# huangzh13/StyleGAN.pytorch

Measured on AMD Instinct MI355X. Metric: img/s full G+D train step, 1024x1024 depth-9 bf16, higher is better.
Workload: dtype bf16; 1 GPU; ffhq1024: StyleGAN 1024x1024, progressive depth index 8, logistic+R1, alpha 0.5, batch 4/GPU, global batch 4; global_batch=4, parallelism=dp1

## Files before the change

stylegan/pytorch_amd/csrc/conv.hip:

```cpp
#include "common.h"
#include <stdlib.h>

enum { G3X3 = 0, GDOWN = 1, GUP = 2, GUPA = 3 };

SGX_SWITCH(conv_percu_cap, "SGX_CONV_PERCU", 0)
SGX_SWITCH(conv_max_ct, "SGX_CONV_MAXCT", 4)
SGX_SWITCH(conv_max_bp, "SGX_CONV_MAXBP", 256)
SGX_SWITCH(conv_min_blocks_env, "SGX_CONV_MINBLOCKS", 0)
SGX_SWITCH(conv_deep_k_on, "SGX_CONV_DEEPK", 1)
SGX_SWITCH(conv_upa_on, "SGX_CONV_UPA", 1)
SGX_SWITCH(conv_splitk_env, "SGX_CONV_SPLITK", 1)
#ifdef SGX_PROBE_BUILD
SGX_SWITCH(conv_dbg, "SGX_CONV_DBG", 0)
#endif

template <typename T, int KC> struct Frag;
template <> struct Frag<float, 16> {
    static constexpr int NK = 4;
    static constexpr int rowb_w() { return 68; }
    static constexpr int rowb_in(int) { return 68; }
    static constexpr bool swz_w() { return false; }
    static constexpr bool swz_in(int) { return false; }
    typedef float frag_t;
    static constexpr int pad_pw(int pw, int) { return pw; }
// ... 574 lines not shown
    }
    SGX_REQUIRE(false, SGX_EINVAL, "conv: bad dtype %d", dtype);
}

__global__ __launch_bounds__(256) void conv_splitk_finish(const float* __restrict__ kws, int ksplit, size_t npix, int Cout, const float* __restrict__ bias,
                                                          int act, const bf16_t* __restrict__ mask, bf16_t* __restrict__ y) {
    const size_t nvec = npix * Cout / 8, stride = npix * Cout;
    const size_t i = (size_t)blockIdx.x * 256 + threadIdx.x;
    if (i >= nvec) return;
    const int c0 = (int)((i * 8) % Cout);
    float v[8];
#pragma unroll
    for (int j = 0; j < 8; ++j) v[j] = 0.f;
    for (int s = 0; s < ksplit; ++s) {
        const float4 a0 = *reinterpret_cast<const float4*>(kws + s * stride + i * 8), a1 = *reinterpret_cast<const float4*>(kws + s * stride + i * 8 + 4);
        v[0] += a0.x; v[1] += a0.y; v[2] += a0.z; v[3] += a0.w; v[4] += a1.x; v[5] += a1.y; v[6] += a1.z; v[7] += a1.w;
    }
    if (bias) {
#pragma unroll
        for (int j = 0; j < 8; ++j) v[j] += bias[c0 + j];
    }
    if (act == SGX_ACT_LRELU) {
#pragma unroll
        for (int j = 0; j < 8; ++j) v[j] = lrelu(v[j]);
    }
    uint4 o = make_uint4(pack_bf16x2(v[0], v[1]), pack_bf16x2(v[2], v[3]), pack_bf16x2(v[4], v[5]), pack_bf16x2(v[6], v[7]));
    if (mask) o = lrelu_mask_bf16x8(o, *reinterpret_cast<const uint4*>(mask + i * 8));
    *reinterpret_cast<uint4*>(y + i * 8) = o;
}
static int conv_splitk_plan(int geo, int B, int H, int W, int Cin, int Cout, int dtype) {
    const int on = conv_splitk_env() < 0 ? 1 : conv_splitk_env();
    if (!on || dtype != SGX_BF16 || geo < 0 || geo > 2 || Cin % 16 || Cout % 16) return 0;
    if (geo != GDOWN) return 0;
    if (sgx_conv2_takes(geo, B, H, W, Cin, Cout)) return 0;
    const int ohc = conv_tile_extent(geo, H), owc = conv_tile_extent(geo, W);
    const bool deep = geo != GDOWN && conv_deep_k(geo, B, ohc, owc, Cin, Cout);
    const ConvCfg c = pick_cfg((geo == GUP && !deep) ? GUPA : geo, B, ohc, owc, Cout);
    if (!c.bp || c.bp > 128 || c.ct > 2 || (deep && c.ct != 1)) return 0;
    const int kc = deep ? 128 : (Cin % 32 == 0 ? 32 : 16);
    const int nk = Cin / kc;
    const long blocks = (long)((B + c.ni - 1) / c.ni) * ((ohc + c.th - 1) / c.th) * ((owc + c.tw - 1) / c.tw) * (Cout / (16 * c.ct)) * ((geo == GUP && deep) ? 4 : 1);
    const int ncu = sgx_ncu();
    if (nk < 4 || blocks > ncu) return 0;
    int want = (int)((2L * ncu + blocks - 1) / blocks);
    const int cap = on > 1 ? on : 8;
    if (want > cap) want = cap;
    if (want > nk / 2) want = nk / 2;
    return want >= 2 ? want : 0;
}
extern "C" size_t sgx_conv_splitk_ws_bytes(int geo, int B, int H, int W, int Cin, int Cout, int dtype) {
    const int ks = conv_splitk_plan(geo, B, H, W, Cin, Cout, dtype);
    if (!ks) return 0;
    const size_t opix = (size_t)B * sgx_conv_out(geo, H) * sgx_conv_out(geo, W);
    return (size_t)ks * opix * Cout * sizeof(float);
}
extern "C" int sgx_conv_splitk(int geo, const void* x, const void* w, const float* bias, void* y, const void* mask, int B, int H, int W, int Cin, int Cout,
                               int act, int dtype, void* ws, size_t ws_bytes, void* stream) {
    const int ks = conv_splitk_plan(geo, B, H, W, Cin, Cout, dtype);
    SGX_REQUIRE(ks > 1, SGX_EUNSUPPORTED, "conv_splitk: this shape does not split (geo %d B%d %dx%d %d->%d)", geo, B, H, W, Cin, Cout);
    SGX_REQUIRE(x && w && y && ws && ws_bytes >= sgx_conv_splitk_ws_bytes(geo, B, H, W, Cin, Cout, dtype), SGX_EWORKSPACE, "conv_splitk: workspace");
    SGX_REQUIRE(geo == G3X3 || !mask, SGX_EINVAL, "conv_splitk: the output mask belongs to the 3x3 geometry");
    SGX_REQUIRE(geo != GDOWN || (H % 2 == 0 && W % 2 == 0), SGX_EINVAL, "conv_splitk: odd input size");
    hipStream_t st = (hipStream_t)stream;
    ConvArgs a = conv_args(geo, x, w, nullptr, y, B, H, W, Cin, Cout, SGX_ACT_NONE);
    a.ksplit = ks; a.kws = static_cast<float*>(ws);
    const int OH = a.OH, OW = a.OW;
    const double taps = geo == G3X3 ? 9.0 : 16.0, opix = (double)B * OH * OW, macs = geo == GUP ? taps / 4.0 : taps;
    SGX_NOTE(2.0 * macs * Cin * Cout * opix, 2.0 * ((double)B * H * W * Cin + opix * Cout + taps * Cin * Cout) + 4.0 * ks * opix * Cout, "conv%c/k%d B%d %dx%d %d->%d",
             geo == G3X3 ? 'S' : (geo == GDOWN ? 'D' : 'U'), ks, B, H, W, Cin, Cout);
    int rc;
    SGX_REQUIRE(geo == GDOWN, SGX_EUNSUPPORTED, "conv_splitk: only the stride-2 geometry has split-K kernels");
    rc = dispatch_conv<GDOWN, true>(a, dtype, st);
    if (rc) return rc;
    const size_t npix = (size_t)B * OH * OW, nvec = npix * Cout / 8;
    SGX_NOTE(0.0, 4.0 * ks * npix * Cout + 2.0 * npix * Cout, "conv_splitk_finish %zux%d", npix, Cout);
    hipLaunchKernelGGL(conv_splitk_finish, dim3((unsigned)((nvec + 255) / 256)), dim3(256), 0, st, (const float*)ws, ks, npix, Cout, bias, act,
                       static_cast<const bf16_t*>(mask), static_cast<bf16_t*>(y));
    SGX_LAUNCH_CHECK("conv_splitk_finish");
    return 0;
}

extern "C" int sgx_conv_config(int geo, int B, int H, int W, int Cin, int Cout, int dtype, int* cfg5) {
    SGX_REQUIRE(geo >= 0 && geo <= 2 && cfg5, SGX_EINVAL, "conv_config: bad args");
    const int ohc = conv_tile_extent(geo, H), owc = conv_tile_extent(geo, W);
    const ConvCfg c = pick_cfg(geo, B, ohc, owc, Cout);
    cfg5[0] = dtype == SGX_F32 ? 16 : (conv_deep_k(geo, B, ohc, owc, Cin, Cout) ? 128 : (Cin % 32 == 0 ? 32 : 16));
    cfg5[1] = c.th; cfg5[2] = c.tw; cfg5[3] = c.bp; cfg5[4] = c.ct;
    return 0;
}

template <int GEO>
static int conv_forward(ConvArgs& a, int dtype, hipStream_t st) {
    if (dtype == SGX_BF16) {
        int launched = 0;
        const int rc = sgx_conv2_try(GEO, a.x, a.w, a.bias, a.y, a.B, a.H, a.W, a.Cin, a.Cout, a.act, a.mask, -1, st, &launched);
        if (rc || launched) return rc;
    }
    return dispatch_conv<GEO>(a, dtype, st);
}

extern "C" int sgx_conv3x3(const void* x, const void* w, const float* bias, void* y, int B, int H, int W, int Cin,
                           int Cout, int act, const void* mask, int dtype, void* stream) {
    ConvArgs a = conv_args(G3X3, x, w, bias, y, B, H, W, Cin, Cout, act);
    a.mask = mask;
    const double es = dtype == SGX_F32 ? 4 : 2;
    SGX_NOTE(2.0 * 9 * Cin * Cout * B * H * W, es * ((double)B * H * W * (Cin + Cout) + 9.0 * Cin * Cout), "convS B%d %dx%d %d->%d", B, H, W, Cin, Cout);
    return conv_forward<G3X3>(a, dtype, (hipStream_t)stream);
}

extern "C" int sgx_conv4x4s2_down(const void* x, const void* w, const float* bias, void* y, int B, int H, int W,
                                  int Cin, int Cout, int act, int dtype, void* stream) {
    SGX_REQUIRE(H % 2 == 0 && W % 2 == 0, SGX_EINVAL, "conv4x4s2_down: odd input size");
    ConvArgs a = conv_args(GDOWN, x, w, bias, y, B, H, W, Cin, Cout, act);
    const double es = dtype == SGX_F32 ? 4 : 2;
    SGX_NOTE(2.0 * 16 * Cin * Cout * B * (H / 2) * (W / 2), es * ((double)B * H * W * (Cin + Cout / 4.0) + 16.0 * Cin * Cout), "convD B%d %dx%d %d->%d", B, H, W, Cin, Cout);
    return conv_forward<GDOWN>(a, dtype, (hipStream_t)stream);
}

extern "C" int sgx_conv4x4s2_up(const void* x, const void* w, void* y, int B, int H, int W, int Cin, int Cout,
                                int dtype, void* stream) {
    ConvArgs a = conv_args(GUP, x, w, nullptr, y, B, H, W, Cin, Cout, SGX_ACT_NONE);
    const double es = dtype == SGX_F32 ? 4 : 2;
    SGX_NOTE(2.0 * 16 * Cin * Cout * B * H * W, es * ((double)B * H * W * (Cin + 4.0 * Cout) + 16.0 * Cin * Cout), "convU B%d %dx%d %d->%d", B, H, W, Cin, Cout);
    return conv_forward<GUP>(a, dtype, (hipStream_t)stream);
}

extern "C" int sgx_conv_variant(int geo, const void* x, const void* w, const float* bias, void* y, int B, int H, int W, int Cin,
                                int Cout, int act, int dtype, int variant, void* stream) {
    SGX_REQUIRE(geo >= 0 && geo <= 2, SGX_EINVAL, "conv_variant: bad geometry %d", geo);
    SGX_REQUIRE(geo != GDOWN || (H % 2 == 0 && W % 2 == 0), SGX_EINVAL, "conv_variant: odd input size");
    SGX_REQUIRE(geo != GUP || (!bias && act == SGX_ACT_NONE), SGX_EINVAL, "conv_variant: the transposed convolution has no fused bias / activation");
    ConvArgs a = conv_args(geo, x, w, bias, y, B, H, W, Cin, Cout, act);
    const int OH = a.OH, OW = a.OW;
    const double es = dtype == SGX_F32 ? 4 : 2, taps = geo == G3X3 ? 9 : 16, npix = (double)B * (geo == GDOWN ? OH * OW : H * W);
    SGX_NOTE(2.0 * taps * Cin * Cout * npix, es * ((double)B * (H * W * Cin + OH * OW * Cout) + taps * Cin * Cout), "conv%c/v%d B%d %dx%d %d->%d", "SDU"[geo], variant, B, H, W, Cin, Cout);
    if (variant == 0) {
        if (geo == G3X3) return dispatch_conv<G3X3>(a, dtype, (hipStream_t)stream);
        if (geo == GDOWN) return dispatch_conv<GDOWN>(a, dtype, (hipStream_t)stream);
        return dispatch_conv<GUP>(a, dtype, (hipStream_t)stream);
    }
    SGX_REQUIRE(dtype == SGX_BF16 && (variant == 4 || variant == 8 || (variant >= 20 && variant <= 29) || (variant >= 30 && variant <= 36)), SGX_EINVAL,
                "conv_variant: variant %d needs bf16 and 4 or 8 waves (or 20..29: a wide-block configuration, 30..36: a conv3_kernel configuration)", variant);
    int launched = 0;
    const int rc = sgx_conv2_try(geo, x, w, bias, y, B, H, W, Cin, Cout, act, nullptr, variant, (hipStream_t)stream, &launched);
    SGX_REQUIRE(rc || launched, SGX_EUNSUPPORTED, "conv_variant: shape not covered by the second-generation kernel");
    return rc;
}

struct WgradArgs {
    const void* kside; const void* nside; float* out;
    int B, Hk, Wk, Hn, Wn, Ck, Cn, tiles_x, tiles_y, ntiles;
    int want_bias;
    int direct; float* dw; float* db; int O, I, mode, transposed, flip_t, accumulate; float scale;
};

template <typename T> struct WFrag;
template <> struct WFrag<float> {
    static constexpr int KPS = 4;
    static constexpr int row_bytes(int ch) { return (ch == 16 ? 16 : ch + 16) * 4; }
    typedef float frag_t;
    __device__ static __forceinline__ frag_t load(const char* base, const int (&poff)[4], int q, int choff) {
        return *reinterpret_cast<const float*>(base + poff[0] + choff * 4);
    }
    __device__ static __forceinline__ f32x4 mma(frag_t a, frag_t b, f32x4 c) {
        return __builtin_amdgcn_mfma_f32_16x16x4f32(a, b, c, 0, 0, 0);
    }
    __device__ static __forceinline__ frag_t ones() { return 1.f; }
};
template <> struct WFrag<bf16_t> {
    static constexpr int KPS = 16;
    static constexpr int row_bytes(int ch) { return ch * 2 + 16; }
    typedef s16x4 frag_t;
    __device__ static __forceinline__ frag_t load(const char* base, const int (&poff)[4], int q, int choff) {
        s16x4 r;
#pragma unroll
        for (int j = 0; j < 4; ++j) r[j] = *reinterpret_cast<const short*>(base + poff[j] + choff * 2);
        return r;
    }
    __device__ static __forceinline__ f32x4 mma(frag_t a, frag_t b, f32x4 c) {
        return __builtin_amdgcn_mfma_f32_16x16x16bf16_1k(a, b, c, 0, 0, 0);
    }
    __device__ static __forceinline__ frag_t ones() { return (s16x4){0x3f80, 0x3f80, 0x3f80, 0x3f80}; }
};

__device__ __forceinline__ s16x4 lds_tr16(const char* p) {
    return __builtin_amdgcn_ds_read_tr16_b64_v4i16((s16x4 __attribute__((address_space(3)))*)(p));
}
__device__ __forceinline__ bf16x8 cat8(s16x4 lo, s16x4 hi) {
    typedef __attribute__((ext_vector_type(8))) short s16x8;
    s16x8 v = __builtin_shufflevector(lo, hi, 0, 1, 2, 3, 4, 5, 6, 7);
    return __builtin_bit_cast(bf16x8, v);
}

template <typename T>
constexpr int wgrad_pitch(int ch, bool tr, int is) {
    return (tr && is == 1) ? (ch == 16 ? 32 : ch * 2 + 32) : WFrag<T>::row_bytes(ch);
}

template <typename T, int GEO, int TH, int TW, int BP, int NSUB, int KSUB, bool TR>
__global__ __launch_bounds__(256) void wgrad_kernel(WgradArgs a) {
    using F = WFrag<T>;
    constexpr int IS = Geo<GEO>::IS, TK = Geo<GEO>::TK, NT = TK * TK;
    constexpr int PH = (TH - 1) * IS + TK, PW = (TW - 1) * IS + TK;
    constexpr int NI = BP / (TH * TW);
    constexpr int NCH = NSUB * 16, KCH = KSUB * 16;
    constexpr int NROW = wgrad_pitch<T>(NCH, TR, 1), KROW = wgrad_pitch<T>(KCH, TR, IS);
    constexpr int VE = 16 / (int)sizeof(T);
    constexpr int TPW = (NT + 3) / 4;
    constexpr int PPL = F::KPS / 4;
    extern __shared__ __attribute__((aligned(16))) char smem[];
    char* n_lds = smem;
    char* k_lds = smem + BP * NROW;

    const int tid = threadIdx.x, lane = tid & 63, wave = tid >> 6, q = lane >> 4, l15 = lane & 15;
    const int kblocks = a.Ck / KCH;
    const int n0 = (blockIdx.x / kblocks) * NCH, kc0 = (blockIdx.x % kblocks) * KCH;
    const T* __restrict__ kg = static_cast<const T*>(a.kside);
    const T* __restrict__ ng = static_cast<const T*>(a.nside);

    f32x4 acc[TPW][NSUB][KSUB];
#pragma unroll
    for (int i = 0; i < TPW; ++i)
#pragma unroll
        for (int j = 0; j < NSUB; ++j)
#pragma unroll
            for (int k = 0; k < KSUB; ++k) acc[i][j][k] = (f32x4){0.f, 0.f, 0.f, 0.f};

    const bool do_bias = a.want_bias && (blockIdx.x % kblocks) == 0 && wave == 3;
    f32x4 bacc[NSUB];
#pragma unroll
    for (int j = 0; j < NSUB; ++j) bacc[j] = (f32x4){0.f, 0.f, 0.f, 0.f};

    constexpr int NNV = (BP * (NCH / VE) + 255) / 256, NKV = (NI * PH * PW * (KCH / VE) + 255) / 256;
    uint4 rn[NNV], rk[NKV];
    auto gload = [&](int tile) {
        int bx = tile;
        const int tx_i = bx % a.tiles_x; bx /= a.tiles_x;
        const int ty_i = bx % a.tiles_y;
        const int img0 = (bx / a.tiles_y) * NI;
        const int ty0 = ty_i * TH, tx0 = tx_i * TW;
        const int iy0 = ty0 * IS - 1, ix0 = tx0 * IS - 1;
#pragma unroll
        for (int j = 0; j < NNV; ++j) {
            const int idx = tid + j * 256;
            const int v = idx % (NCH / VE), m = idx / (NCH / VE);
            const int il = m / (TH * TW), r = (m / TW) % TH, c = m % TW;
            const int b = img0 + il, gy = ty0 + r, gx = tx0 + c;
            const bool ok = (idx < BP * (NCH / VE)) && (b < a.B) && (gy < a.Hn) && (gx < a.Wn);
            const T* src = ng + (((size_t)b * a.Hn + gy) * a.Wn + gx) * a.Cn + n0 + v * VE;
            rn[j] = ok ? *reinterpret_cast<const uint4*>(src) : make_uint4(0, 0, 0, 0);
        }
#pragma unroll
        for (int j = 0; j < NKV; ++j) {
            const int idx = tid + j * 256;
            const int v = idx % (KCH / VE), pixel = idx / (KCH / VE);
            const int il = pixel / (PH * PW), rem = pixel % (PH * PW);
            const int gy = iy0 + rem / PW, gx = ix0 + rem % PW, b = img0 + il;
            const bool ok = (idx < NI * PH * PW * (KCH / VE)) && (b < a.B) && ((unsigned)gy < (unsigned)a.Hk) && ((unsigned)gx < (unsigned)a.Wk);
            const T* src = kg + (((size_t)b * a.Hk + gy) * a.Wk + gx) * a.Ck + kc0 + v * VE;
            rk[j] = ok ? *reinterpret_cast<const uint4*>(src) : make_uint4(0, 0, 0, 0);
        }
    };
    auto lstore = [&]() {
#pragma unroll
        for (int j = 0; j < NNV; ++j) {
            const int idx = tid + j * 256;
            if (idx < BP * (NCH / VE)) *reinterpret_cast<uint4*>(n_lds + (idx / (NCH / VE)) * NROW + (idx % (NCH / VE)) * 16) = rn[j];
        }
#pragma unroll
        for (int j = 0; j < NKV; ++j) {
            const int idx = tid + j * 256;
            if (idx < NI * PH * PW * (KCH / VE)) *reinterpret_cast<uint4*>(k_lds + (idx / (KCH / VE)) * KROW + (idx % (KCH / VE)) * 16) = rk[j];
        }
    };
    if ((int)blockIdx.y < a.ntiles) gload(blockIdx.y);
    for (int tile = blockIdx.y; tile < a.ntiles; tile += gridDim.y) {
        __syncthreads();
        lstore();
        __syncthreads();
        if (tile + (int)gridDim.y < a.ntiles) gload(tile + gridDim.y);
        if constexpr (TR) {
            for (int ks = 0; ks < BP / 32; ++ks) {
                int noff2[2], koff2[2];
#pragma unroll
                for (int h = 0; h < 2; ++h) {
                    const int m = ks * 32 + h * 16 + q * 4 + (l15 >> 2);
                    const int il = m / (TH * TW), r = (m / TW) % TH, c = m % TW;
                    noff2[h] = m * NROW + (l15 & 3) * 8;
                    koff2[h] = ((il * PH + r * IS) * PW + c * IS) * KROW + (l15 & 3) * 8;
                }
                bf16x8 fa8[NSUB];
#pragma unroll
                for (int ns = 0; ns < NSUB; ++ns)
                    fa8[ns] = cat8(lds_tr16(n_lds + noff2[0] + ns * 32), lds_tr16(n_lds + noff2[1] + ns * 32));
                if (do_bias) {
                    const bf16x8 one8 = cat8(WFrag<bf16_t>::ones(), WFrag<bf16_t>::ones());
#pragma unroll
                    for (int ns = 0; ns < NSUB; ++ns) bacc[ns] = __builtin_amdgcn_mfma_f32_16x16x32_bf16(fa8[ns], one8, bacc[ns], 0, 0, 0);
                }
#pragma unroll
                for (int i = 0; i < TPW; ++i) {
                    const int t = wave + 4 * i;
                    if (t < NT) {
                        const int toff = ((t / TK) * PW + (t % TK)) * KROW;
#pragma unroll
                        for (int kk = 0; kk < KSUB; ++kk) {
                            const bf16x8 fb8 = cat8(lds_tr16(k_lds + toff + koff2[0] + kk * 32), lds_tr16(k_lds + toff + koff2[1] + kk * 32));
#pragma unroll
                            for (int ns = 0; ns < NSUB; ++ns)
                                acc[i][ns][kk] = __builtin_amdgcn_mfma_f32_16x16x32_bf16(fa8[ns], fb8, acc[i][ns][kk], 0, 0, 0);
                        }
                    }
                }
            }
        } else
        for (int ks = 0; ks < BP / F::KPS; ++ks) {
            int noff[4], koff[4];
#pragma unroll
            for (int j = 0; j < PPL; ++j) {
                const int m = ks * F::KPS + q * PPL + j;
                const int il = m / (TH * TW), r = (m / TW) % TH, c = m % TW;
                noff[j] = m * NROW;
                koff[j] = ((il * PH + r * IS) * PW + c * IS) * KROW;
            }
            typename F::frag_t fa[NSUB];
#pragma unroll
            for (int ns = 0; ns < NSUB; ++ns) fa[ns] = F::load(n_lds, noff, q, ns * 16 + l15);
            if (do_bias) {
#pragma unroll
                for (int ns = 0; ns < NSUB; ++ns) bacc[ns] = F::mma(fa[ns], F::ones(), bacc[ns]);
            }
#pragma unroll
            for (int i = 0; i < TPW; ++i) {
                const int t = wave + 4 * i;
                if (t < NT) {
                    const int toff = ((t / TK) * PW + (t % TK)) * KROW;
#pragma unroll
                    for (int kk = 0; kk < KSUB; ++kk) {
                        typename F::frag_t fb = F::load(k_lds + toff, koff, q, kk * 16 + l15);
#pragma unroll
                        for (int ns = 0; ns < NSUB; ++ns) acc[i][ns][kk] = F::mma(fa[ns], fb, acc[i][ns][kk]);
                    }
                }
            }
        }
    }
    if (a.direct) {
        constexpr int KP = KCH + 1;
        float* accl = reinterpret_cast<float*>(smem);
        __syncthreads();
#pragma unroll
        for (int i = 0; i < TPW; ++i) {
            const int t = wave + 4 * i;
            if (t < NT) {
#pragma unroll
                for (int ns = 0; ns < NSUB; ++ns)
#pragma unroll
                    for (int kk = 0; kk < KSUB; ++kk)
#pragma unroll
                        for (int r = 0; r < 4; ++r) accl[(t * NCH + ns * 16 + q * 4 + r) * KP + kk * 16 + l15] = acc[i][ns][kk][r];
            }
        }
        __syncthreads();
        const float c = a.scale * (a.mode == SGX_PACK_D ? 0.25f : 1.f);
        for (int idx = tid; idx < NCH * KCH * 9; idx += 256) {
            const int tap = idx % 9, kl = (idx / 9) % KCH, nl = idx / (9 * KCH);
            const int n = n0 + nl, k = kc0 + kl;
            const int o = a.transposed ? k : n, i = a.transposed ? n : k;
            if (i >= a.I || o >= a.O) continue;
            float v;
            if (NT == 9) {
                v = accl[((a.flip_t ? 8 - tap : tap) * NCH + nl) * KP + kl];
            } else {
                const int y = tap / 3, x = tap % 3;
                const float* pp = accl + nl * KP + kl;
                v = (pp[(y * 4 + x) * NCH * KP] + pp[(y * 4 + x + 1) * NCH * KP]) +
                    (pp[((y + 1) * 4 + x) * NCH * KP] + pp[((y + 1) * 4 + x + 1) * NCH * KP]);
            }
            float* d = a.dw + ((size_t)o * a.I + i) * 9 + (a.mode == SGX_PACK_UF ? 8 - tap : tap);
            *d = (a.accumulate & 1) ? *d + c * v : c * v;
        }
        if (do_bias && l15 == 0) {
#pragma unroll
            for (int ns = 0; ns < NSUB; ++ns)
#pragma unroll
                for (int r = 0; r < 4; ++r) {
                    float* d = a.db + n0 + ns * 16 + q * 4 + r;
                    *d = (a.accumulate & 2) ? *d + bacc[ns][r] : bacc[ns][r];
                }
        }
        return;
    }
    float* out = a.out + (size_t)blockIdx.y * ((size_t)NT * a.Cn * a.Ck + a.Cn);
    if (do_bias && l15 == 0) {
#pragma unroll
        for (int ns = 0; ns < NSUB; ++ns)
#pragma unroll
            for (int r = 0; r < 4; ++r) out[(size_t)NT * a.Cn * a.Ck + n0 + ns * 16 + q * 4 + r] = bacc[ns][r];
    }
#pragma unroll
    for (int i = 0; i < TPW; ++i) {
        const int t = wave + 4 * i;
        if (t < NT) {
#pragma unroll
            for (int ns = 0; ns < NSUB; ++ns)
#pragma unroll
                for (int kk = 0; kk < KSUB; ++kk)
#pragma unroll
                    for (int r = 0; r < 4; ++r)
                        out[((size_t)t * a.Cn + n0 + ns * 16 + q * 4 + r) * a.Ck + kc0 + kk * 16 + l15] = acc[i][ns][kk][r];
        }
    }
}

struct FinishArgs { const float* ws; float* dw; float* db; int nsplit, O, I, Ip, mode, transposed, flip_t; float scale; int accumulate; };

template <int EPB>
__global__ __launch_bounds__(256) void wgrad_finish_kernel(FinishArgs f) {
    constexpr int NSL = 256 / EPB;
    __shared__ float red[NSL][EPB][9];
    const int pl = threadIdx.x % EPB, sl = threadIdx.x / EPB;
    const int A = f.transposed ? f.Ip : f.O, Bd = f.transposed ? f.O : f.Ip;
    const int e = blockIdx.x * EPB + pl;
    const int taps = f.mode == SGX_PACK_S ? 9 : 16;
    const size_t tstride = (size_t)f.O * f.Ip, total = (size_t)taps * tstride + A;
    if ((int)blockIdx.x >= (A * Bd + EPB - 1) / EPB) {
        const int o = ((int)blockIdx.x - (A * Bd + EPB - 1) / EPB) * EPB + pl;
        float b = 0.f;
        if (o < f.O)
            for (int s = sl; s < f.nsplit; s += NSL) b += f.ws[(size_t)s * total + (size_t)taps * tstride + o];
        red[sl][pl][0] = b;
        __syncthreads();
        if (sl == 0 && o < f.O) {
            float sum = 0.f;
            for (int l = 0; l < NSL; ++l) sum += red[l][pl][0];
            f.db[o] = (f.accumulate & 2) ? f.db[o] + sum : sum;
        }
        return;
    }
    float acc[9];
#pragma unroll
    for (int k = 0; k < 9; ++k) acc[k] = 0.f;
    if (e < A * Bd) {
#pragma unroll 4
        for (int s = sl; s < f.nsplit; s += NSL) {
            const float* p = f.ws + (size_t)s * total + e;
            if (f.mode == SGX_PACK_S) {
#pragma unroll
                for (int t = 0; t < 9; ++t) acc[t] += p[(size_t)(f.flip_t ? 8 - t : t) * tstride];
            } else {
                float v[16];
#pragma unroll
                for (int t = 0; t < 16; ++t) v[t] = p[(size_t)t * tstride];
#pragma unroll
                for (int y = 0; y < 3; ++y)
#pragma unroll
                    for (int x = 0; x < 3; ++x)
                        acc[y * 3 + x] += (v[y * 4 + x] + v[y * 4 + x + 1]) + (v[(y + 1) * 4 + x] + v[(y + 1) * 4 + x + 1]);
            }
        }
    }
#pragma unroll
    for (int k = 0; k < 9; ++k) red[sl][pl][k] = acc[k];
    __syncthreads();
    for (int t = threadIdx.x; t < EPB * 9; t += 256) {
        const int el = t / 9, k = t % 9;
        const int ee = blockIdx.x * EPB + el;
        if (ee >= A * Bd) continue;
        const int a = ee / Bd, bb = ee % Bd;
        const int o = f.transposed ? bb : a, i = f.transposed ? a : bb;
        if (i >= f.I) continue;
        float sum = 0.f;
#pragma unroll 8
        for (int l = 0; l < NSL; ++l) sum += red[l][el][k];
        const float c = f.scale * (f.mode == SGX_PACK_D ? 0.25f : 1.f);
        float* d = f.dw + ((size_t)o * f.I + i) * 9 + (f.mode == SGX_PACK_UF ? 8 - k : k);
        *d = (f.accumulate & 1) ? *d + c * sum : c * sum;
    }
}

static int wgrad_nsplit(int pairs, int ntiles, size_t elems_per_split) {
    static const int env_target = [] { const char* e = getenv("SGX_WGRAD_BLOCKS"); return e && atoi(e) > 0 ? atoi(e) : 0; }();
    static const int env_cap = [] { const char* e = getenv("SGX_WGRAD_MAXSPLIT"); return e && atoi(e) > 0 ? atoi(e) : 0; }();
    const bool tiny = elems_per_split <= (size_t)16 * 32 * 32;
    static const int env_mid = [] { const char* e = getenv("SGX_WGRAD_BLOCKS_MID"); return e && atoi(e) > 0 ? atoi(e) : 0; }();
    const int target = env_target ? env_target : (tiny ? 2048 : (env_mid ? env_mid : 512)), cap = env_cap ? env_cap : (tiny ? 1024 : 512);
    int want = (target + pairs - 1) / pairs;
    if (!env_target && pairs >= 512 && ntiles <= 64) want = 1;
    if (want > cap) want = cap;
    if (want > ntiles) want = ntiles;
    if (want < 1) want = 1;
    return want;
}

template <typename T, int GEO, int TH, int TW, int BP, int NSUB, int KSUB, bool TR>
static int launch_wgrad(WgradArgs& a, void* ws, size_t ws_bytes, int* nsplit_out, hipStream_t st) {
    using F = WFrag<T>;
    constexpr int IS = Geo<GEO>::IS, TK = Geo<GEO>::TK, NT = TK * TK;
    constexpr int PH = (TH - 1) * IS + TK, PW = (TW - 1) * IS + TK, NI = BP / (TH * TW);
    constexpr int OPER = BP * wgrad_pitch<T>(NSUB * 16, TR, 1) + NI * PH * PW * wgrad_pitch<T>(KSUB * 16, TR, IS);
    constexpr int FOLD = NT * NSUB * 16 * (KSUB * 16 + 1) * 4;
    constexpr int LDS = OPER > FOLD ? OPER : FOLD;
    static_assert(LDS <= 160 * 1024, "LDS budget");
    a.tiles_y = (a.Hn + TH - 1) / TH; a.tiles_x = (a.Wn + TW - 1) / TW;
    a.ntiles = ((a.B + NI - 1) / NI) * a.tiles_y * a.tiles_x;
    const int pairs = (a.Cn / (NSUB * 16)) * (a.Ck / (KSUB * 16));
    int nsplit = wgrad_nsplit(pairs, a.ntiles, (size_t)NT * a.Cn * a.Ck);
    const size_t total = (size_t)NT * a.Cn * a.Ck + a.Cn;
    size_t fit = ws_bytes / (total * sizeof(float));
    if ((size_t)nsplit > fit) nsplit = (int)fit;
    SGX_REQUIRE(nsplit >= 1, SGX_EWORKSPACE, "wgrad: workspace too small (%zu bytes, need >= %zu)", ws_bytes, total * sizeof(float));
    a.out = static_cast<float*>(ws);
    a.direct = (nsplit == 1 && a.dw != nullptr) ? 1 : 0;
    auto kern = wgrad_kernel<T, GEO, TH, TW, BP, NSUB, KSUB, TR>;
    sgx_lds_opt_in<wgrad_kernel<T, GEO, TH, TW, BP, NSUB, KSUB, TR>>(LDS);
    hipLaunchKernelGGL(kern, dim3(pairs, nsplit), dim3(256), LDS, st, a);
    SGX_LAUNCH_CHECK("wgrad_kernel");
    *nsplit_out = nsplit;
    return 0;
}

template <typename T, int GEO, int BP, int NSUB, int KSUB, bool TR>
static int wgrad_tile(WgradArgs& a, void* ws, size_t wsb, int* ns, hipStream_t st) {
    if (a.Hn >= 16 && a.Wn >= 16) return launch_wgrad<T, GEO, BP / 16, 16, BP, NSUB, KSUB, TR>(a, ws, wsb, ns, st);
    if (a.Hn >= 8 && a.Wn >= 8) return launch_wgrad<T, GEO, (BP >= 64 ? 8 : BP / 8), 8, BP, NSUB, KSUB, TR>(a, ws, wsb, ns, st);
    return launch_wgrad<T, GEO, (BP >= 16 ? 4 : BP / 4), 4, BP, NSUB, KSUB, TR>(a, ws, wsb, ns, st);
}

static bool wgrad_use_tr() {
    static const int v = [] { const char* e = getenv("SGX_WGRAD_TR"); return e ? atoi(e) : 1; }();
    return v != 0;
}

template <typename T, int GEO, int BP, bool TR = false>
static int wgrad_ch(WgradArgs& a, void* ws, size_t wsb, int* ns, hipStream_t st) {
    SGX_REQUIRE(a.Cn % 16 == 0 && a.Ck % 16 == 0, SGX_EUNSUPPORTED, "wgrad: channels must be multiples of 16");
    const bool n32 = a.Cn % 32 == 0, k32 = a.Ck % 32 == 0;
    if (GEO == GDOWN) {
        if (n32) return wgrad_tile<T, GEO, BP, 2, 1, TR>(a, ws, wsb, ns, st);
        return wgrad_tile<T, GEO, BP, 1, 1, TR>(a, ws, wsb, ns, st);
    }
    const long npix = (long)a.B * a.Hn * a.Wn;
    const bool lowres_big = npix <= 64L * BP && (long)(a.Cn / 32) * (a.Ck / 32) < 512 && (long)(a.Cn / 32) * (a.Ck / 16) >= 512;
    if (n32 && k32 && !lowres_big) return wgrad_tile<T, GEO, BP, 2, 2, TR>(a, ws, wsb, ns, st);
    if (n32) return wgrad_tile<T, GEO, BP, 2, 1, TR>(a, ws, wsb, ns, st);
    if (k32) return wgrad_tile<T, GEO, BP, 1, 2, TR>(a, ws, wsb, ns, st);
    return wgrad_tile<T, GEO, BP, 1, 1, TR>(a, ws, wsb, ns, st);
}

static int wgrad_pre_groups() { static const int v = [] { const char* e = getenv("SGX_WGRAD_PRE"); return e ? atoi(e) : 32; }(); return v; }
static int wgrad_pre_min() { static const int v = [] { const char* e = getenv("SGX_WGRAD_PRE_MIN"); return e ? atoi(e) : 256; }(); return v; }
__global__ __launch_bounds__(256) void wgrad_prereduce_kernel(const float* __restrict__ ws, float* __restrict__ out, size_t total4,
                                                              int nsplit) {
    const size_t e = (size_t)blockIdx.x * 256 + threadIdx.x;
    if (e >= total4) return;
    const int g = blockIdx.y, per = (nsplit + (int)gridDim.y - 1) / (int)gridDim.y;
    const int s0 = g * per, s1 = (s0 + per < nsplit) ? s0 + per : nsplit;
    float4 acc = make_float4(0.f, 0.f, 0.f, 0.f);
#pragma unroll 4
    for (int sp = s0; sp < s1; ++sp) {
        const float4 v = reinterpret_cast<const float4*>(ws)[(size_t)sp * total4 + e];
        acc.x += v.x; acc.y += v.y; acc.z += v.z; acc.w += v.w;
    }
    reinterpret_cast<float4*>(out)[(size_t)g * total4 + e] = acc;
}
static size_t wgrad_pre_bytes(size_t total_floats, int nsplit) {
    const int G = wgrad_pre_groups();
    return (G > 0 && nsplit >= wgrad_pre_min() && nsplit > G && total_floats % 4 == 0) ? (size_t)G * total_floats * sizeof(float) : 0;
}

static int wgrad_finish(const void* ws, float* dw, float* db, int nsplit, int O, int I, int Ip, int mode, int transposed, int flip_t,
                        float scale, int accumulate, hipStream_t st, size_t ws_bytes = 0) {
    {
        const size_t total = (size_t)(mode == SGX_PACK_S ? 9 : 16) * O * Ip + (transposed ? Ip : O);
        const size_t pre = wgrad_pre_bytes(total, nsplit), used = (size_t)nsplit * total * sizeof(float);
        if (pre && ws_bytes >= used + pre) {
            float* out = reinterpret_cast<float*>(const_cast<char*>(static_cast<const char*>(ws)) + used);
            hipLaunchKernelGGL(wgrad_prereduce_kernel, dim3((unsigned)((total / 4 + 255) / 256), wgrad_pre_groups()), dim3(256), 0, st,
                               static_cast<const float*>(ws), out, total / 4, nsplit);
            SGX_LAUNCH_CHECK("wgrad_prereduce_kernel");
            ws = out;
            nsplit = wgrad_pre_groups();
        }
    }
    FinishArgs f{static_cast<const float*>(ws), dw, db, nsplit, O, I, Ip, mode, transposed, flip_t, scale, accumulate};
    SGX_NOTE(0.0, 4.0 * ((double)nsplit * (mode == SGX_PACK_S ? 9 : 16) * O * Ip + 9.0 * O * I), "finish %dx%d m%d tr%d ns%d", O, I, mode, transposed, nsplit);
    const int ne = O * Ip, nb = db ? O : 0;
    if (ne / 64 >= 128) hipLaunchKernelGGL(wgrad_finish_kernel<64>, dim3((unsigned)((ne + 63) / 64 + (nb + 63) / 64)), dim3(256), 0, st, f);
    else if (ne / 16 >= 128) hipLaunchKernelGGL(wgrad_finish_kernel<16>, dim3((unsigned)((ne + 15) / 16 + (nb + 15) / 16)), dim3(256), 0, st, f);
    else if (ne / 8 >= 128) hipLaunchKernelGGL(wgrad_finish_kernel<8>, dim3((unsigned)((ne + 7) / 8 + (nb + 7) / 8)), dim3(256), 0, st, f);
    else hipLaunchKernelGGL(wgrad_finish_kernel<4>, dim3((unsigned)((ne + 3) / 4 + (nb + 3) / 4)), dim3(256), 0, st, f);
    SGX_LAUNCH_CHECK("wgrad_finish_kernel");
    return 0;
}

extern "C" size_t sgx_wgrad_ws_bytes(int taps, int B, int H, int W, int Ck, int Cn) {
    size_t total = ((size_t)taps * Ck * Cn + Cn) * sizeof(float);
    int pairs = (Ck / 32 > 0 ? Ck / 32 : 1) * (Cn / 32 > 0 ? Cn / 32 : 1);
    size_t ntiles = (size_t)B * ((H + 3) / 4) * ((W + 3) / 4);
    size_t ns = (size_t)wgrad_nsplit(pairs, ntiles > (1u << 30) ? (1 << 30) : (int)ntiles, (size_t)taps * Ck * Cn);
    size_t need = total * ns + wgrad_pre_bytes(total / sizeof(float), (int)ns);
    int a0, a1, a2, a3;
    const int ns2 = taps == 9 ? sgx_wgrad2_plan(0, B, H, W, Ck, Cn, &a0, &a1, &a2, &a3) : sgx_wgrad2_plan(1, B, H / 2, W / 2, Ck, Cn, &a0, &a1, &a2, &a3);
    const size_t need2 = ns2 ? total * ns2 + wgrad_pre_bytes(total / sizeof(float), ns2) : 0;
    return need > need2 ? need : need2;
}

extern "C" int sgx_wgrad3x3_param(const void* x, const void* dy, float* dW, float* db, void* ws, size_t ws_bytes, int B, int H,
                                  int W, int Cx, int Cdy, int adjoint, float scale, int O, int I, int accumulate, int dtype,
                                  void* stream) {
    hipStream_t st = (hipStream_t)stream;
    const int Ip = adjoint ? Cdy : Cx;
    SGX_REQUIRE(!db || !adjoint, SGX_EINVAL, "wgrad3x3_param: bias gradient asked of the adjoint launch");
    SGX_REQUIRE((adjoint ? Cx : Cdy) == O && Ip >= I, SGX_EINVAL, "wgrad3x3_param: channel mismatch (Cx=%d Cdy=%d O=%d I=%d adj=%d)", Cx, Cdy, O, I, adjoint);
    WgradArgs a{x, dy, nullptr, B, H, W, H, W, Cx, Cdy, 0, 0, 0, db ? 1 : 0,
                0, dW, db, O, I, SGX_PACK_S, adjoint, adjoint, accumulate, scale};
    SGX_NOTE(2.0 * 9 * Cx * Cdy * B * H * W, (dtype == SGX_F32 ? 4.0 : 2.0) * B * H * W * (Cx + Cdy), "wgradS B%d %dx%d %dx%d", B, H, W, Cx, Cdy);
    int ns = 0, rc;
    if (dtype == SGX_BF16) {
        rc = sgx_wgrad2_launch(0, x, dy, static_cast<float*>(ws), ws_bytes, B, H, W, Cx, Cdy, db ? 1 : 0, st, &ns);
        if (rc) return rc;
        if (ns) return wgrad_finish(ws, dW, db, ns, O, I, Ip, SGX_PACK_S, adjoint, adjoint, scale, accumulate, st, ws_bytes);
    }
    if (dtype == SGX_F32) rc = wgrad_ch<float, G3X3, 128>(a, ws, ws_bytes, &ns, st);
    else if (dtype == SGX_BF16) rc = wgrad_use_tr() ? wgrad_ch<bf16_t, G3X3, 128, true>(a, ws, ws_bytes, &ns, st) : wgrad_ch<bf16_t, G3X3, 128>(a, ws, ws_bytes, &ns, st);
    else { SGX_REQUIRE(false, SGX_EINVAL, "wgrad3x3_param: bad dtype"); }
    if (rc) return rc;
    if (a.direct) return 0;
    return wgrad_finish(ws, dW, db, ns, O, I, Ip, SGX_PACK_S, adjoint, adjoint, scale, accumulate, st, ws_bytes);
}

extern "C" int sgx_wgrad4x4s2_param(const void* fine, const void* coarse, float* dW, float* db, void* ws, size_t ws_bytes, int B,
                                    int H, int W, int Cfine, int Ccoarse, int mode, float scale, int O, int I, int accumulate,
                                    int dtype, void* stream) {
    hipStream_t st = (hipStream_t)stream;
    SGX_REQUIRE(H % 2 == 0 && W % 2 == 0, SGX_EINVAL, "wgrad4x4s2_param: odd fine size");
    SGX_REQUIRE(mode == SGX_PACK_D || mode == SGX_PACK_U || mode == SGX_PACK_UF, SGX_EINVAL, "wgrad4x4s2_param: bad mode %d", mode);
    const int transposed = mode != SGX_PACK_D;
    SGX_REQUIRE(!db || !transposed, SGX_EINVAL, "wgrad4x4s2_param: bias gradient only for mode D (dy is the coarse side)");
    SGX_REQUIRE(transposed ? (Ccoarse == I && Cfine == O) : (Ccoarse == O && Cfine == I), SGX_EINVAL,
                "wgrad4x4s2_param: channel mismatch (fine %d coarse %d O %d I %d mode %d)", Cfine, Ccoarse, O, I, mode);
    WgradArgs a{fine, coarse, nullptr, B, H, W, H / 2, W / 2, Cfine, Ccoarse, 0, 0, 0, db ? 1 : 0,
                0, dW, db, O, I, mode, transposed, 0, accumulate, scale};
    SGX_NOTE(2.0 * 16 * Cfine * Ccoarse * B * (H / 2) * (W / 2), (dtype == SGX_F32 ? 4.0 : 2.0) * B * H * W * (Cfine + Ccoarse / 4.0), "wgradD B%d fine%dx%d %dx%d", B, H, W, Cfine, Ccoarse);
    int ns = 0, rc;
    if (dtype == SGX_BF16) {
        rc = sgx_wgrad2_launch(1, fine, coarse, static_cast<float*>(ws), ws_bytes, B, H / 2, W / 2, Cfine, Ccoarse, db ? 1 : 0, st, &ns);
        if (rc) return rc;
        if (ns) return wgrad_finish(ws, dW, db, ns, O, I, I, mode, transposed, 0, scale, accumulate, st, ws_bytes);
    }
    if (dtype == SGX_F32) rc = wgrad_ch<float, GDOWN, 64>(a, ws, ws_bytes, &ns, st);
    else if (dtype == SGX_BF16) rc = wgrad_use_tr() ? wgrad_ch<bf16_t, GDOWN, 64, true>(a, ws, ws_bytes, &ns, st) : wgrad_ch<bf16_t, GDOWN, 64>(a, ws, ws_bytes, &ns, st);
    else { SGX_REQUIRE(false, SGX_EINVAL, "wgrad4x4s2_param: bad dtype"); }
    if (rc) return rc;
    if (a.direct) return 0;
    return wgrad_finish(ws, dW, db, ns, O, I, I, mode, transposed, 0, scale, accumulate, st, ws_bytes);
}

#define PACK_T 32
__device__ __forceinline__ float pack_tap(const float (*raw)[PACK_T][PACK_T + 1], int r, int il, int t, int mode, float scale) {
    if (mode == SGX_PACK_S) return scale * raw[t][r][il];
    const int ky = t >> 2, kx = t & 3;
    float v = 0.f;
#pragma unroll
    for (int a = 0; a < 2; ++a)
#pragma unroll
        for (int b = 0; b < 2; ++b) {
            const int y = ky - a, x = kx - b;
            if (y >= 0 && y < 3 && x >= 0 && x < 3) v += raw[mode == SGX_PACK_UF ? (2 - y) * 3 + (2 - x) : y * 3 + x][r][il];
// ... 112 lines not shown
```

Baseline: 281.7 img/s.

## Add register-ring prefetch and double-buffered LDS to transposed wgrad kernel

For the transposed-read bf16 weight-gradient kernel, global loads for upcoming tiles are kept in a ring of register stages (depth two for 3x3 single-subtile configs), and LDS can alternate between two buffers when the per-CU LDS budget allows, removing one barrier per tile. Tile coordinates are advanced incrementally, bounds-failing loads are redirected to a safe address and masked afterward, and B fragments are optionally batch-loaded before the MFMA loop. This aims to hide global load latency and cut sync stalls, at the cost of more registers and LDS, which can lower occupancy.

```diff
diff --git a/stylegan/pytorch_amd/csrc/conv.hip b/stylegan/pytorch_amd/csrc/conv.hip
--- a/stylegan/pytorch_amd/csrc/conv.hip
+++ b/stylegan/pytorch_amd/csrc/conv.hip
@@ -750,6 +750,7 @@
     int B, Hk, Wk, Hn, Wn, Ck, Cn, tiles_x, tiles_y, ntiles;
     int want_bias;
     int direct; float* dw; float* db; int O, I, mode, transposed, flip_t, accumulate; float scale;
+    int lds_stages;
 };
 
 template <typename T> struct WFrag;
@@ -793,6 +794,13 @@
 template <typename T>
 constexpr int wgrad_pitch(int ch, bool tr, int is) {
     return (tr && is == 1) ? (ch == 16 ? 32 : ch * 2 + 32) : WFrag<T>::row_bytes(ch);
+}
+
+template <typename T, int GEO, int TW, int NSUB, int KSUB, bool TR>
+constexpr int wgrad_ring() {
+    if (!TR) return 0;
+    if (GEO == G3X3 && NSUB * KSUB == 1) return 2;
+    return 1;
 }
 
 template <typename T, int GEO, int TH, int TW, int BP, int NSUB, int KSUB, bool TR>
@@ -830,54 +838,117 @@
     for (int j = 0; j < NSUB; ++j) bacc[j] = (f32x4){0.f, 0.f, 0.f, 0.f};
 
     constexpr int NNV = (BP * (NCH / VE) + 255) / 256, NKV = (NI * PH * PW * (KCH / VE) + 255) / 256;
-    uint4 rn[NNV], rk[NKV];
-    auto gload = [&](int tile) {
-        int bx = tile;
-        const int tx_i = bx % a.tiles_x; bx /= a.tiles_x;
-        const int ty_i = bx % a.tiles_y;
-        const int img0 = (bx / a.tiles_y) * NI;
-        const int ty0 = ty_i * TH, tx0 = tx_i * TW;
-        const int iy0 = ty0 * IS - 1, ix0 = tx0 * IS - 1;
-#pragma unroll
-        for (int j = 0; j < NNV; ++j) {
+    constexpr int D = wgrad_ring<T, GEO, TW, NSUB, KSUB, TR>();
+    if constexpr (D == 0) {
+        uint4 rn[NNV], rk[NKV];
+        auto gload = [&](int tile) {
+            int bx = tile;
+            const int tx_i = bx % a.tiles_x; bx /= a.tiles_x;
+            const int ty_i = bx % a.tiles_y;
+            const int img0 = (bx / a.tiles_y) * NI;
+            const int ty0 = ty_i * TH, tx0 = tx_i * TW;
+            const int iy0 = ty0 * IS - 1, ix0 = tx0 * IS - 1;
+#pragma unroll
+            for (int j = 0; j < NNV; ++j) {
+                const int idx = tid + j * 256;
+                const int v = idx % (NCH / VE), m = idx / (NCH / VE);
+                const int il = m / (TH * TW), r = (m / TW) % TH, c = m % TW;
+                const int b = img0 + il, gy = ty0 + r, gx = tx0 + c;
+                const bool ok = (idx < BP * (NCH / VE)) && (b < a.B) && (gy < a.Hn) && (gx < a.Wn);
+                const T* src = ng + (((size_t)b * a.Hn + gy) * a.Wn + gx) * a.Cn + n0 + v * VE;
+                rn[j] = ok ? *reinterpret_cast<const uint4*>(src) : make_uint4(0, 0, 0, 0);
+            }
+#pragma unroll
+            for (int j = 0; j < NKV; ++j) {
+                const int idx = tid + j * 256;
+                const int v = idx % (KCH / VE), pixel = idx / (KCH / VE);
+                const int il = pixel / (PH * PW), rem = pixel % (PH * PW);
+                const int gy = iy0 + rem / PW, gx = ix0 + rem % PW, b = img0 + il;
+                const bool ok = (idx < NI * PH * PW * (KCH / VE)) && (b < a.B) && ((unsigned)gy < (unsigned)a.Hk) && ((unsigned)gx < (unsigned)a.Wk);
+                const T* src = kg + (((size_t)b * a.Hk + gy) * a.Wk + gx) * a.Ck + kc0 + v * VE;
+                rk[j] = ok ? *reinterpret_cast<const uint4*>(src) : make_uint4(0, 0, 0, 0);
+            }
+        };
+        auto lstore = [&]() {
+#pragma unroll
+            for (int j = 0; j < NNV; ++j) {
+                const int idx = tid + j * 256;
+                if (idx < BP * (NCH / VE)) *reinterpret_cast<uint4*>(n_lds + (idx / (NCH / VE)) * NROW + (idx % (NCH / VE)) * 16) = rn[j];
+            }
+#pragma unroll
+            for (int j = 0; j < NKV; ++j) {
+                const int idx = tid + j * 256;
+                if (idx < NI * PH * PW * (KCH / VE)) *reinterpret_cast<uint4*>(k_lds + (idx / (KCH / VE)) * KROW + (idx % (KCH / VE)) * 16) = rk[j];
+            }
+        };
+        if ((int)blockIdx.y < a.ntiles) gload(blockIdx.y);
+        for (int tile = blockIdx.y; tile < a.ntiles; tile += gridDim.y) {
+            __syncthreads();
+            lstore();
+            __syncthreads();
+            if (tile + (int)gridDim.y < a.ntiles) gload(tile + gridDim.y);
+            for (int ks = 0; ks < BP / F::KPS; ++ks) {
+                int noff[4], koff[4];
+#pragma unroll
+                for (int j = 0; j < PPL; ++j) {
+                    const int m = ks * F::KPS + q * PPL + j;
+                    const int il = m / (TH * TW), r = (m / TW) % TH, c = m % TW;
+                    noff[j] = m * NROW;
+                    koff[j] = ((il * PH + r * IS) * PW + c * IS) * KROW;
+                }
+                typename F::frag_t fa[NSUB];
+#pragma unroll
+                for (int ns = 0; ns < NSUB; ++ns) fa[ns] = F::load(n_lds, noff, q, ns * 16 + l15);
+                if (do_bias) {
+#pragma unroll
+                    for (int ns = 0; ns < NSUB; ++ns) bacc[ns] = F::mma(fa[ns], F::ones(), bacc[ns]);
+                }
+#pragma unroll
+                for (int i = 0; i < TPW; ++i) {
+                    const int t = wave + 4 * i;
+                    if (t < NT) {
+                        const int toff = ((t / TK) * PW + (t % TK)) * KROW;
+#pragma unroll
+                        for (int kk = 0; kk < KSUB; ++kk) {
+                            typename F::frag_t fb = F::load(k_lds + toff, koff, q, kk * 16 + l15);
+#pragma unroll
+                            for (int ns = 0; ns < NSUB; ++ns) acc[i][ns][kk] = F::mma(fa[ns], fb, acc[i][ns][kk]);
+                        }
+                    }
+                }
+            }
+        }
+    } else {
+        auto n_src = [&](int j, int tx_i, int ty_i, int img0, bool& ok) __attribute__((always_inline)) {
             const int idx = tid + j * 256;
             const int v = idx % (NCH / VE), m = idx / (NCH / VE);
             const int il = m / (TH * TW), r = (m / TW) % TH, c = m % TW;
-            const int b = img0 + il, gy = ty0 + r, gx = tx0 + c;
-            const bool ok = (idx < BP * (NCH / VE)) && (b < a.B) && (gy < a.Hn) && (gx < a.Wn);
-            const T* src = ng + (((size_t)b * a.Hn + gy) * a.Wn + gx) * a.Cn + n0 + v * VE;
-            rn[j] = ok ? *reinterpret_cast<const uint4*>(src) : make_uint4(0, 0, 0, 0);
-        }
-#pragma unroll
-        for (int j = 0; j < NKV; ++j) {
+            const int b = img0 + il, gy = ty_i * TH + r, gx = tx_i * TW + c;
+            ok = (idx < BP * (NCH / VE)) && (b < a.B) && (gy < a.Hn) && (gx < a.Wn);
+            return ng + (((size_t)b * a.Hn + gy) * a.Wn + gx) * a.Cn + n0 + v * VE;
+        };
+        auto k_src = [&](int j, int tx_i, int ty_i, int img0, bool& ok) __attribute__((always_inline)) {
             const int idx = tid + j * 256;
             const int v = idx % (KCH / VE), pixel = idx / (KCH / VE);
             const int il = pixel / (PH * PW), rem = pixel % (PH * PW);
-            const int gy = iy0 + rem / PW, gx = ix0 + rem % PW, b = img0 + il;
-            const bool ok = (idx < NI * PH * PW * (KCH / VE)) && (b < a.B) && ((unsigned)gy < (unsigned)a.Hk) && ((unsigned)gx < (unsigned)a.Wk);
-            const T* src = kg + (((size_t)b * a.Hk + gy) * a.Wk + gx) * a.Ck + kc0 + v * VE;
-            rk[j] = ok ? *reinterpret_cast<const uint4*>(src) : make_uint4(0, 0, 0, 0);
-        }
-    };
-    auto lstore = [&]() {
-#pragma unroll
-        for (int j = 0; j < NNV; ++j) {
-            const int idx = tid + j * 256;
-            if (idx < BP * (NCH / VE)) *reinterpret_cast<uint4*>(n_lds + (idx / (NCH / VE)) * NROW + (idx % (NCH / VE)) * 16) = rn[j];
-        }
-#pragma unroll
-        for (int j = 0; j < NKV; ++j) {
-            const int idx = tid + j * 256;
-            if (idx < NI * PH * PW * (KCH / VE)) *reinterpret_cast<uint4*>(k_lds + (idx / (KCH / VE)) * KROW + (idx % (KCH / VE)) * 16) = rk[j];
-        }
-    };
-    if ((int)blockIdx.y < a.ntiles) gload(blockIdx.y);
-    for (int tile = blockIdx.y; tile < a.ntiles; tile += gridDim.y) {
-        __syncthreads();
-        lstore();
-        __syncthreads();
-        if (tile + (int)gridDim.y < a.ntiles) gload(tile + gridDim.y);
-        if constexpr (TR) {
+            const int gy = ty_i * TH * IS - 1 + rem / PW, gx = tx_i * TW * IS - 1 + rem % PW, b = img0 + il;
+            ok = (idx < NI * PH * PW * (KCH / VE)) && (b < a.B) && ((unsigned)gy < (unsigned)a.Hk) && ((unsigned)gx < (unsigned)a.Wk);
+            return kg + (((size_t)b * a.Hk + gy) * a.Wk + gx) * a.Ck + kc0 + v * VE;
+        };
+        auto lstore = [&](const uint4 (&rn)[NNV], const uint4 (&rk)[NKV], char* n_lds, char* k_lds) __attribute__((always_inline)) {
+#pragma unroll
+            for (int j = 0; j < NNV; ++j) {
+                const int idx = tid + j * 256;
+                if (idx < BP * (NCH / VE)) *reinterpret_cast<uint4*>(n_lds + (idx / (NCH / VE)) * NROW + (idx % (NCH / VE)) * 16) = rn[j];
+            }
+#pragma unroll
+            for (int j = 0; j < NKV; ++j) {
+                const int idx = tid + j * 256;
+                if (idx < NI * PH * PW * (KCH / VE)) *reinterpret_cast<uint4*>(k_lds + (idx / (KCH / VE)) * KROW + (idx % (KCH / VE)) * 16) = rk[j];
+            }
+        };
+        constexpr bool BATCH = !(GEO == G3X3 && NSUB == 1 && KSUB == 2) && !(GEO == GDOWN && TW == 8 && NSUB == 2);
+        auto mma_tile = [&](const char* n_lds, const char* k_lds) __attribute__((always_inline)) {
             for (int ks = 0; ks < BP / 32; ++ks) {
                 int noff2[2], koff2[2];
 #pragma unroll
@@ -887,10 +958,20 @@
                     noff2[h] = m * NROW + (l15 & 3) * 8;
                     koff2[h] = ((il * PH + r * IS) * PW + c * IS) * KROW + (l15 & 3) * 8;
                 }
-                bf16x8 fa8[NSUB];
+                bf16x8 fa8[NSUB], fb8[TPW][KSUB];
 #pragma unroll
                 for (int ns = 0; ns < NSUB; ++ns)
                     fa8[ns] = cat8(lds_tr16(n_lds + noff2[0] + ns * 32), lds_tr16(n_lds + noff2[1] + ns * 32));
+                auto k_frag = [&](int t, int kk) __attribute__((always_inline)) {
+                    const int toff = ((t / TK) * PW + (t % TK)) * KROW;
+                    return cat8(lds_tr16(k_lds + toff + koff2[0] + kk * 32), lds_tr16(k_lds + toff + koff2[1] + kk * 32));
+                };
+                if constexpr (BATCH) {
+#pragma unroll
+                    for (int i = 0; i < TPW; ++i)
+#pragma unroll
+                        for (int kk = 0; kk < KSUB; ++kk) fb8[i][kk] = k_frag(wave + 4 * i < NT ? wave + 4 * i : wave, kk);
+                }
                 if (do_bias) {
                     const bf16x8 one8 = cat8(WFrag<bf16_t>::ones(), WFrag<bf16_t>::ones());
 #pragma unroll
@@ -898,50 +979,64 @@
                 }
 #pragma unroll
                 for (int i = 0; i < TPW; ++i) {
-                    const int t = wave + 4 * i;
-                    if (t < NT) {
-                        const int toff = ((t / TK) * PW + (t % TK)) * KROW;
+                    if (wave + 4 * i < NT) {
 #pragma unroll
                         for (int kk = 0; kk < KSUB; ++kk) {
-                            const bf16x8 fb8 = cat8(lds_tr16(k_lds + toff + koff2[0] + kk * 32), lds_tr16(k_lds + toff + koff2[1] + kk * 32));
+                            if constexpr (!BATCH) fb8[i][kk] = k_frag(wave + 4 * i, kk);
 #pragma unroll
                             for (int ns = 0; ns < NSUB; ++ns)
-                                acc[i][ns][kk] = __builtin_amdgcn_mfma_f32_16x16x32_bf16(fa8[ns], fb8, acc[i][ns][kk], 0, 0, 0);
+                                acc[i][ns][kk] = __builtin_amdgcn_mfma_f32_16x16x32_bf16(fa8[ns], fb8[i][kk], acc[i][ns][kk], 0, 0, 0);
                         }
                     }
                 }
             }
-        } else
-        for (int ks = 0; ks < BP / F::KPS; ++ks) {
-            int noff[4], koff[4];
-#pragma unroll
-            for (int j = 0; j < PPL; ++j) {
-                const int m = ks * F::KPS + q * PPL + j;
-                const int il = m / (TH * TW), r = (m / TW) % TH, c = m % TW;
-                noff[j] = m * NROW;
-                koff[j] = ((il * PH + r * IS) * PW + c * IS) * KROW;
-            }
-            typename F::frag_t fa[NSUB];
-#pragma unroll
-            for (int ns = 0; ns < NSUB; ++ns) fa[ns] = F::load(n_lds, noff, q, ns * 16 + l15);
-            if (do_bias) {
-#pragma unroll
-                for (int ns = 0; ns < NSUB; ++ns) bacc[ns] = F::mma(fa[ns], F::ones(), bacc[ns]);
-            }
-#pragma unroll
-            for (int i = 0; i < TPW; ++i) {
-                const int t = wave + 4 * i;
-                if (t < NT) {
-                    const int toff = ((t / TK) * PW + (t % TK)) * KROW;
-#pragma unroll
-                    for (int kk = 0; kk < KSUB; ++kk) {
-                        typename F::frag_t fb = F::load(k_lds + toff, koff, q, kk * 16 + l15);
-#pragma unroll
-                        for (int ns = 0; ns < NSUB; ++ns) acc[i][ns][kk] = F::mma(fa[ns], fb, acc[i][ns][kk]);
-                    }
-                }
-            }
-        }
+        };
+        constexpr int OPER = BP * NROW + NI * PH * PW * KROW, NV = NNV + NKV;
+        uint4 rn[D][NNV], rk[D][NKV];
+        unsigned okm[D];
+        const int nwalk = ((int)blockIdx.y < a.ntiles) ? (a.ntiles - 1 - (int)blockIdx.y) / (int)gridDim.y + 1 : 0;
+        const int txy = a.tiles_x * a.tiles_y;
+        const int sx = (int)gridDim.y % a.tiles_x, sy = ((int)gridDim.y / a.tiles_x) % a.tiles_y, si = (int)gridDim.y / txy;
+        int tx = (int)blockIdx.y % a.tiles_x, ty = ((int)blockIdx.y / a.tiles_x) % a.tiles_y, im = (int)blockIdx.y / txy;
+        auto gload = [&](uint4 (&rn)[NNV], uint4 (&rk)[NKV], unsigned& okm) __attribute__((always_inline)) {
+            unsigned m = 0;
+#pragma unroll
+            for (int j = 0; j < NV; ++j) {
+                bool ok;
+                const T* p = j < NNV ? n_src(j, tx, ty, im * NI, ok) : k_src(j - NNV, tx, ty, im * NI, ok);
+                (j < NNV ? rn[j] : rk[j - NNV]) = *reinterpret_cast<const uint4*>(ok ? p : (j < NNV ? ng : kg));
+                m |= ok ? 1u << j : 0u;
+            }
+            okm = m;
+            tx += sx; ty += sy; im += si;
+            if (tx >= a.tiles_x) { tx -= a.tiles_x; ++ty; }
+            if (ty >= a.tiles_y) { ty -= a.tiles_y; ++im; }
+        };
+        const int stage = a.lds_stages == 2 ? OPER : 0;
+#pragma unroll
+        for (int s = 0; s < D; ++s) {
+            gload(rn[s], rk[s], okm[s]);
+            __builtin_amdgcn_sched_barrier(0);
+        }
+        auto step = [&](uint4 (&rn)[NNV], uint4 (&rk)[NKV], unsigned& okm, int j) __attribute__((always_inline)) {
+            char* nb = smem + (j & 1) * stage;
+            if (stage == 0) __syncthreads();
+#pragma unroll
+            for (int v = 0; v < NNV; ++v) if (!((okm >> v) & 1u)) rn[v] = make_uint4(0, 0, 0, 0);
+#pragma unroll
+            for (int v = 0; v < NKV; ++v) if (!((okm >> (NNV + v)) & 1u)) rk[v] = make_uint4(0, 0, 0, 0);
+            lstore(rn, rk, nb, nb + BP * NROW);
+            __syncthreads();
+            gload(rn, rk, okm);
+            mma_tile(nb, nb + BP * NROW);
+        };
+        int j = 0;
+        for (; j + D <= nwalk; j += D) {
+#pragma unroll
+            for (int s = 0; s < D; ++s) step(rn[s], rk[s], okm[s], j + s);
+        }
+#pragma unroll
+        for (int s = 0; s + 1 < D; ++s) if (j + s < nwalk) step(rn[s], rk[s], okm[s], j + s);
     }
     if (a.direct) {
         constexpr int KP = KCH + 1;
@@ -1111,8 +1206,16 @@
     a.out = static_cast<float*>(ws);
     a.direct = (nsplit == 1 && a.dw != nullptr) ? 1 : 0;
     auto kern = wgrad_kernel<T, GEO, TH, TW, BP, NSUB, KSUB, TR>;
-    sgx_lds_opt_in<wgrad_kernel<T, GEO, TH, TW, BP, NSUB, KSUB, TR>>(LDS);
-    hipLaunchKernelGGL(kern, dim3(pairs, nsplit), dim3(256), LDS, st, a);
+    constexpr bool RING = wgrad_ring<T, GEO, TW, NSUB, KSUB, TR>() > 0;
+    constexpr int LDS2 = RING && 2 * OPER > FOLD ? 2 * OPER : LDS;
+    static_assert(LDS2 <= 160 * 1024, "LDS budget");
+    long per_cu = ((long)pairs * nsplit + sgx_ncu() - 1) / sgx_ncu();
+    if (per_cu > 8) per_cu = 8;
+    const bool two = RING && a.ntiles > nsplit && per_cu * LDS2 <= 160 * 1024;
+    a.lds_stages = two ? 2 : 1;
+    const int lds = two ? LDS2 : LDS;
+    sgx_lds_opt_in<wgrad_kernel<T, GEO, TH, TW, BP, NSUB, KSUB, TR>>(LDS2);
+    hipLaunchKernelGGL(kern, dim3(pairs, nsplit), dim3(256), lds, st, a);
     SGX_LAUNCH_CHECK("wgrad_kernel");
     *nsplit_out = nsplit;
     return 0;
```

New measurement: 281.4 img/s. No clear change (-0.1%).
